# LongmaoTeamTf/deep_recommenders

Measured on AMD Instinct MI355X. Metric: examples/sec/node DeepFM (26 sparse feats, 10M vocab, dim 64), higher is better.
Workload: dtype f32; 1 GPU; DeepFM Criteo-shape synthetic training step (BASELINE.json configs[2]): 26 sparse + 13 dense, 10000000 vocab/field hashed on device, dim 64, DNN [256, 32]+[1] relu, sigmoid-CE, fused SGD; batch 65536 per GPU, ids uniform; tables on one GPU (66.6 GB); gemm_split=f16x2, global_batch=65536, parallelism=single, per_kernel_events=False

## Files before the change

deep_recommenders_amd/csrc/bf3_wgrad.hip:

```cpp
#ifndef DR_NT_WGRAD_GATHER
#define DR_NT_WGRAD_GATHER 0
#endif
#include "bf3_rs_core.h"
#include "tn_rs_reduce.h"

namespace {

using namespace drrs;

struct TnRsArgs {
    const float* X; int64_t ldx;
    const float* Y; int64_t ldy;
    int64_t R; int32_t F; int32_t N;
    int64_t per; int32_t split;
    float* partial; float* colsum;
    const int32_t* ids_t; const int64_t* row_base; const float* table; int32_t nf; const float* dense_pad;
    const uint32_t* x_amax; const uint32_t* x2_amax; const uint32_t* y_amax;
    uint32_t* hdr;
};

template <int GATHER, int H2 = 0>
__global__ __launch_bounds__(512, 2) void bf3_gemm_tn_rs_kernel(TnRsArgs g) {
    constexpr int NW = 8, BMF = 32 * NW, BN = 256, NT = BN / 32;
    constexpr int NPL = RS_NPL<H2>, B_PLANE = RS_B_PLANE, STAGE = RS_STAGE<H2>;
    __shared__ __attribute__((aligned(1024))) unsigned char smem[2 * STAGE];

    const int tid = threadIdx.x, lane = tid & 63;
    const int wave = __builtin_amdgcn_readfirstlane(tid >> 6);
    const int l31 = lane & 31, hi = lane >> 5;
    const int tiles_n = (g.N + BN - 1) / BN, tiles_f = (g.F + BMF - 1) / BMF;
    const int per_slice = tiles_f * tiles_n;
    const int Fp = tiles_f * BMF, Np = tiles_n * BN;
    const int lid = xcd_remap(blockIdx.x, per_slice * g.split);
    const int slice = lid / per_slice, t = lid % per_slice;
    const int f0 = (t / tiles_n) * BMF, n0 = (t % tiles_n) * BN;
    const int64_t r_begin = (int64_t)slice * g.per;
    int64_t r_end = r_begin + g.per;
    if (r_end > g.R) r_end = g.R;
    const int nk = (int)((r_end - r_begin + BK - 1) / BK);
    const bool want_cs = g.colsum != nullptr && f0 == 0;
    float h2_sx = 1.f, h2_sy = 1.f;
    if constexpr (H2) {
        float inv;
        h2_prologue(g.x_amax, g.x2_amax, g.y_amax, h2_sx, h2_sy, inv);
        if (lid == 0 && tid == 0) {
            g.hdr[0] = max(g.x_amax[0], g.x2_amax != nullptr ? g.x2_amax[0] : 0u);
            g.hdr[1] = g.y_amax[0];
        }
    }

    const int fcol = min(f0 + wave * 32 + l31, g.F - 1);
    const int ncol = min(n0 + wave * 32 + l31, g.N - 1);
    const unsigned lds0 = (unsigned)(uintptr_t)(lds_ptr_t)smem;
    const int sw = tn_img_swizzle(l31);
    unsigned b_addr[2];
#pragma unroll
    for (int s = 0; s < 2; ++s) b_addr[s] = rs_frag_addr(lds0, l31, hi, sw, s);
    unsigned char* const wrow = smem + (wave * 32 + l31) * 64;

    float xa[16], yb[16];
    const unsigned xoff = (unsigned)((16 * hi * g.ldx + fcol) * 4), yoff = (unsigned)((16 * hi * g.ldy + ncol) * 4);
    auto load_raw = [&](float (&dst)[16], const float* base, int64_t ld, unsigned voff, int64_t r0) {
        if (r0 + BK <= r_end) {
            const char* rowp = reinterpret_cast<const char*>(base + r0 * ld);
#pragma unroll
            for (int e = 0; e < 16; ++e) dst[e] = *reinterpret_cast<const float*>(rowp + (int64_t)e * ld * 4 + voff);
        } else {
#pragma unroll
            for (int e = 0; e < 16; ++e) {
                const int64_t r = r0 + 16 * hi + e;
                const bool ok = r < r_end;
                const float v = *reinterpret_cast<const float*>(reinterpret_cast<const char*>(base + (ok ? r : r_end - 1) * ld) +
                                                                (voff - (unsigned)(16 * hi * ld * 4)));
                dst[e] = ok ? v : 0.f;
            }
        }
    };
    const int c0w = f0 + wave * 32;
    const bool w_field = GATHER && c0w < 64 * g.nf;
    const bool w_dense = GATHER && !w_field && g.dense_pad != nullptr && c0w < 64 * g.nf + 32;
    const float* gptr = g.table;
    unsigned gpitch = 0;
    const int32_t* idrow = nullptr;
    if (GATHER) {
        if (w_field) {
            const int fld = c0w >> 6;
            const int64_t rbv = g.row_base[fld];
            const int64_t rb = (int64_t)(((uint64_t)(uint32_t)__builtin_amdgcn_readfirstlane((int)(rbv >> 32)) << 32) |
                                         (uint32_t)__builtin_amdgcn_readfirstlane((int)rbv));
            gptr = g.table + rb * 64 + (c0w & 32);
            gpitch = 256;
            idrow = g.ids_t + (int64_t)fld * g.R;
        } else if (w_dense) {
            gptr = g.dense_pad;
            gpitch = 128;
        }
    }
    const __amdgpu_buffer_rsrc_t grsrc =
        __builtin_amdgcn_make_buffer_rsrc(const_cast<float*>(gptr), 0, (w_field || w_dense) ? (int)0xFFFFFF00u : 0, 0x00020000);
    const unsigned gcol = (unsigned)l31 * 4u;
    const int id_lane = (lane & 15) + 16 * hi;
    int idv = 0;
    auto gather_id = [&](int ids_of_tile, int e) -> int {
        switch (e) {
#define GATHER_ID(E) case E: return __builtin_amdgcn_update_dpp(0, ids_of_tile, 0x150 + E, 0xf, 0xf, false);
            GATHER_ID(0) GATHER_ID(1) GATHER_ID(2) GATHER_ID(3) GATHER_ID(4) GATHER_ID(5) GATHER_ID(6) GATHER_ID(7)
            GATHER_ID(8) GATHER_ID(9) GATHER_ID(10) GATHER_ID(11) GATHER_ID(12) GATHER_ID(13) GATHER_ID(14)
#undef GATHER_ID
            default: return __builtin_amdgcn_update_dpp(0, ids_of_tile, 0x15f, 0xf, 0xf, false);
        }
    };
    auto load_ids = [&](int64_t r0) -> int {
        if (!w_field) return 0;
        const int64_t r = r0 + id_lane < g.R ? r0 + id_lane : g.R - 1;
        return idrow[r];
    };
    auto load_gather = [&](float (&dst)[16], int ids_of_tile, int64_t r0) {
        const bool full = r0 + BK <= r_end;
        unsigned off[16];
        if (w_field) {
#pragma unroll
            for (int e = 0; e < 16; ++e) off[e] = (unsigned)gather_id(ids_of_tile, e) * gpitch;
        } else {
            const unsigned o0 = (unsigned)(r0 + 16 * hi) * gpitch;
#pragma unroll
            for (int e = 0; e < 16; ++e) off[e] = o0 + (unsigned)e * gpitch;
        }
        if (!full) {
            const int nv = (int)(r_end - r0 < BK ? r_end - r0 : BK) - 16 * hi;
#pragma unroll
            for (int e = 0; e < 16; ++e) off[e] = e < nv ? off[e] : 0xFFFFFF00u;
        }
#pragma unroll
        for (int e = 0; e < 16; ++e)
            dst[e] = __builtin_bit_cast(float, __builtin_amdgcn_raw_buffer_load_b32(grsrc, (int)(off[e] + gcol), 0, DR_NT_WGRAD_GATHER ? 2 : 0));
    };
    bf16x8 fa[2][3];
    bf16x8 fb[4][3];
    float cs = 0.f;
    auto stage_b = [&](int stage) {
        if (want_cs) {
#pragma unroll
            for (int e = 0; e < 16; ++e) cs += yb[e];
        }
#pragma unroll
        for (int s = 0; s < 2; ++s) {
            bf16x8 p0, p1, p2;
            float v[8];
#pragma unroll
            for (int j = 0; j < 8; ++j) v[j] = yb[8 * s + j];
            if constexpr (H2) h2_split8v(v, h2_sy, p0, p1);
            else rs_split8v(v, p0, p1, p2);
            unsigned char* w = wrow + stage * STAGE + rs_chunk_off(hi, sw, s);
            *reinterpret_cast<bf16x8*>(w) = p0;
            *reinterpret_cast<bf16x8*>(w + B_PLANE) = p1;
            if constexpr (!H2) *reinterpret_cast<bf16x8*>(w + 2 * B_PLANE) = p2;
        }
    };
    auto read_b = [&](int buf, int stage, int q) {
        const unsigned bb = b_addr[q >> 3] + stage * STAGE;
        rs_read_frag<NPL>(fb[buf], bb, q & 7);
    };
    f32x16 acc[NT];
#pragma unroll
    for (int tt = 0; tt < NT; ++tt)
#pragma unroll
        for (int k = 0; k < 16; ++k) acc[tt][k] = 0.f;

    load_raw(yb, g.Y, g.ldy, yoff, r_begin);
    stage_b(0);
    if (GATHER) {
        idv = load_ids(r_begin);
        load_gather(xa, idv, r_begin);
        idv = load_ids(r_begin + BK);
    } else {
        load_raw(xa, g.X, g.ldx, xoff, r_begin);
    }
    load_raw(yb, g.Y, g.ldy, yoff, r_begin + BK);
    asm volatile("s_waitcnt lgkmcnt(0)\n\ts_barrier" ::: "memory");
    read_b(0, 0, 0);
    read_b(1, 0, 1);

    for (int kt = 0; kt < nk; ++kt) {
        const int stage = kt & 1;
        {
            float v[8];
#pragma unroll
            for (int s = 0; s < 2; ++s) {
#pragma unroll
                for (int j = 0; j < 8; ++j) v[j] = xa[8 * s + j];
                if constexpr (H2) h2_split8v(v, h2_sx, fa[s][0], fa[s][1]);
                else rs_split8v(v, fa[s][0], fa[s][1], fa[s][2]);
            }
        }
        if (kt + 1 < nk) stage_b(stage ^ 1);
        __builtin_amdgcn_sched_barrier(0);
        if (GATHER) {
            load_gather(xa, idv, r_begin + (int64_t)(kt + 1) * BK);
            idv = load_ids(r_begin + (int64_t)(kt + 2) * BK);
        } else {
            load_raw(xa, g.X, g.ldx, xoff, r_begin + (int64_t)(kt + 1) * BK);
        }
        load_raw(yb, g.Y, g.ldy, yoff, r_begin + (int64_t)(kt + 2) * BK);
        __builtin_amdgcn_sched_barrier(0);
#pragma unroll
        for (int q = 0; q < 16; ++q) {
            if (q < 14) {
                rs_wait_frag<NPL, NPL>(fb[q & 3]);
                read_b((q + 2) & 3, stage, q + 2);
            } else if (q == 14) {
                rs_wait_frag<NPL, 0>(fb[2]);
                asm volatile("s_barrier" ::: "memory");
                if (kt + 1 < nk) read_b(0, stage ^ 1, 0);
            } else {
                if (kt + 1 < nk) read_b(1, stage ^ 1, 1);
            }
            __builtin_amdgcn_sched_barrier(0);
#pragma unroll
            for (int term = 0; term < RS_TERMS<H2>; ++term) acc[q & 7] = rs_mma_term<H2>(term, fa[q >> 3], fb[q & 3], acc[q & 7]);
            __builtin_amdgcn_sched_barrier(0);
        }
    }
    float* out = g.partial + ((int64_t)slice * Fp + f0 + wave * 32 + 4 * hi) * Np + n0 + l31;
#pragma unroll
    for (int nt = 0; nt < NT; ++nt)
#pragma unroll
        for (int reg = 0; reg < 16; ++reg) out[(int64_t)((reg & 3) + 8 * (reg >> 2)) * Np + nt * 32] = acc[nt][reg];
    if (want_cs) {
        cs += __shfl_xor(cs, 32, 64);
        if (hi == 0) g.colsum[(int64_t)slice * Np + n0 + wave * 32 + l31] = cs;
    }
}

template <int V>
__global__ __launch_bounds__(TN_RS_RED_THREADS) void bf3_tn_rs_reduce_kernel(TnRsApply a) {
    tn_rs_reduce_block<V>(a, blockIdx.x, threadIdx.x);
}

void launch_tn_rs_reduce(const TnRsApply& a, dr_stream_t stream) {
    const int nlb = tn_rs_reduce_blocks(a.F, a.N, a.vec);
    if (a.vec) hipLaunchKernelGGL(bf3_tn_rs_reduce_kernel<4>, dim3(nlb), dim3(TN_RS_RED_THREADS), 0, dr_s(stream), a);
    else hipLaunchKernelGGL(bf3_tn_rs_reduce_kernel<1>, dim3(nlb), dim3(TN_RS_RED_THREADS), 0, dr_s(stream), a);
}
}

void drrs::tn_rs_plan(int64_t R, int32_t F, int32_t N, int& split, int64_t& per, int& Fp, int& Np) {
    const int tf = (F + 255) / 256, tn = (N + 255) / 256;
    Fp = tf * 256;
    Np = tn * 256;
    int64_t sp = 256 / ((int64_t)tf * tn);
    const int64_t max_split = (R + 16 * BK - 1) / (16 * BK);
    if (sp > max_split) sp = max_split;
    if (sp < 1) sp = 1;
    per = ((R + sp - 1) / sp + BK - 1) / BK * BK;
    split = (int)((R + per - 1) / per);
}

extern "C" int64_t dr_bf3_wgrad_workspace_bytes(int64_t R, int32_t F, int32_t N) {
    if (R <= 0 || F <= 0 || N <= 0) return 0;
    int split, Fp, Np;
    int64_t per;
    tn_rs_plan(R, F, N, split, per, Fp, Np);
    return ((int64_t)split * Fp * Np + (int64_t)split * Np + TN_RS_HDR_WORDS) * (int64_t)sizeof(float);
}

static int wgrad_impl(const float* x, int64_t ld_x, const float* dy, int64_t ld_dy, int64_t R, int32_t F, int32_t N,
                      float scale, float* dstW, int64_t ld_w, float* dstb, void* workspace, int64_t workspace_bytes,
                      dr_stream_t stream, const uint32_t* x_amax = nullptr, const uint32_t* dy_amax = nullptr) {
    if (R <= 0 || F <= 0 || N <= 0) return DR_EINVAL;
    if (!x || !dy || !dstW || !workspace || ld_x < F || ld_dy < N || ld_w < N) return DR_EINVAL;
    if (workspace_bytes < dr_bf3_wgrad_workspace_bytes(R, F, N)) return DR_EINVAL;
    int split, Fp, Np;
    int64_t per;
    tn_rs_plan(R, F, N, split, per, Fp, Np);
    const bool h2 = x_amax != nullptr;
    const TnRsApply ap = tn_rs_apply_of(workspace, split, F, N, Fp, Np, h2, scale, dstW, ld_w, dstb);
    TnRsArgs g{x, ld_x, dy, ld_dy, R, F, N, per, split, const_cast<float*>(ap.partial), const_cast<float*>(ap.colsum), nullptr, nullptr, nullptr, 0,
               nullptr, x_amax, nullptr, dy_amax, const_cast<uint32_t*>(ap.hdr)};
    const int grid = (Fp / 256) * (Np / 256) * split;
    if (h2) hipLaunchKernelGGL((bf3_gemm_tn_rs_kernel<0, 1>), dim3(grid), dim3(512), 0, dr_s(stream), g);
    else hipLaunchKernelGGL((bf3_gemm_tn_rs_kernel<0, 0>), dim3(grid), dim3(512), 0, dr_s(stream), g);
    launch_tn_rs_reduce(ap, stream);
    DR_CHECK_LAUNCH();
    return DR_OK;
}

extern "C" int dr_bf3_wgrad(const float* x, int64_t ld_x, const float* dy, int64_t ld_dy, int64_t R, int32_t F, int32_t N,
                            float scale, float* dstW, int64_t ld_w, float* dstb, void* workspace, int64_t workspace_bytes,
                            dr_stream_t stream) {
    return wgrad_impl(x, ld_x, dy, ld_dy, R, F, N, scale, dstW, ld_w, dstb, workspace, workspace_bytes, stream);
}

extern "C" int dr_h2_wgrad(const float* x, int64_t ld_x, const uint32_t* x_amax, const float* dy, int64_t ld_dy, const uint32_t* dy_amax,
                           int64_t R, int32_t F, int32_t N, float scale, float* dstW, int64_t ld_w, float* dstb, void* workspace,
                           int64_t workspace_bytes, dr_stream_t stream) {
    if (!x_amax || !dy_amax) return DR_EINVAL;
    return wgrad_impl(x, ld_x, dy, ld_dy, R, F, N, scale, dstW, ld_w, dstb, workspace, workspace_bytes, stream, x_amax, dy_amax);
}

static int wgrad_emb_impl(const int32_t* ids_t, int64_t R, int32_t nf, const int64_t* row_base, const float* table, int32_t D,
                          const float* dense_pad, const float* dy, int64_t ld_dy, int32_t F, int32_t N, float scale, float* dstW,
                          int64_t ld_w, float* dstb, void* workspace, int64_t workspace_bytes, int32_t parts, dr_stream_t stream,
                          const uint32_t* table_amax = nullptr, const uint32_t* dense_amax = nullptr, const uint32_t* dy_amax = nullptr) {
    if (R <= 0 || F <= 0 || N <= 0 || nf <= 0) return DR_EINVAL;
    if (table_amax != nullptr && (!dy_amax || (F > 64 * nf && !dense_amax))) return DR_EINVAL;
    if (D != 64 || F < 64 * nf || F > 64 * nf + 32) return DR_ESHAPE;
    if (!ids_t || !row_base || !table || !dy || !dstW || !workspace || ld_dy < N || ld_w < N) return DR_EINVAL;
    if (F > 64 * nf && !dense_pad) return DR_EINVAL;
    if (workspace_bytes < dr_bf3_wgrad_workspace_bytes(R, F, N)) return DR_EINVAL;
    int split, Fp, Np;
    int64_t per;
    tn_rs_plan(R, F, N, split, per, Fp, Np);
    const bool h2 = table_amax != nullptr;
    const TnRsApply ap = tn_rs_apply_of(workspace, split, F, N, Fp, Np, h2, scale, dstW, ld_w, dstb);
    TnRsArgs g{nullptr, 0, dy, ld_dy, R, F, N, per, split, const_cast<float*>(ap.partial), const_cast<float*>(ap.colsum), ids_t, row_base, table,
               nf, F > 64 * nf ? dense_pad : nullptr, table_amax, F > 64 * nf ? dense_amax : nullptr, dy_amax, const_cast<uint32_t*>(ap.hdr)};
    const int grid = (Fp / 256) * (Np / 256) * split;
    if (parts & 1) {
        if (h2) hipLaunchKernelGGL((bf3_gemm_tn_rs_kernel<1, 1>), dim3(grid), dim3(512), 0, dr_s(stream), g);
        else hipLaunchKernelGGL((bf3_gemm_tn_rs_kernel<1, 0>), dim3(grid), dim3(512), 0, dr_s(stream), g);
    }
    if (parts & 2) launch_tn_rs_reduce(ap, stream);
    DR_CHECK_LAUNCH();
    return DR_OK;
}

extern "C" int dr_bf3_wgrad_emb(const int32_t* ids_t, int64_t R, int32_t nf, const int64_t* row_base, const float* table, int32_t D,
                                const float* dense_pad, const float* dy, int64_t ld_dy, int32_t F, int32_t N, float scale, float* dstW,
                                int64_t ld_w, float* dstb, void* workspace, int64_t workspace_bytes, int32_t parts, dr_stream_t stream) {
    if (parts < 1 || parts > 3) return DR_EINVAL;
    return wgrad_emb_impl(ids_t, R, nf, row_base, table, D, dense_pad, dy, ld_dy, F, N, scale, dstW, ld_w, dstb, workspace, workspace_bytes,
                          parts, stream);
}

extern "C" int dr_h2_wgrad_emb(const int32_t* ids_t, int64_t R, int32_t nf, const int64_t* row_base, const float* table, int32_t D,
                               const uint32_t* table_amax, const float* dense_pad, const uint32_t* dense_amax, const float* dy, int64_t ld_dy,
                               const uint32_t* dy_amax, int32_t F, int32_t N, float scale, float* dstW, int64_t ld_w, float* dstb,
                               void* workspace, int64_t workspace_bytes, int32_t parts, dr_stream_t stream) {
    if (parts < 1 || parts > 3 || !table_amax || !dy_amax) return DR_EINVAL;
    return wgrad_emb_impl(ids_t, R, nf, row_base, table, D, dense_pad, dy, ld_dy, F, N, scale, dstW, ld_w, dstb, workspace, workspace_bytes,
                          parts, stream, table_amax, dense_amax, dy_amax);
}
```

Baseline: 75.08 million examples/sec.

## Interleave A/B global loads and splits into MFMA groups for f16x2 wgrad path

For the H2 (f16x2) variant of the TN reduce-scatter wgrad GEMM, the main loop runs over full K tiles with unguarded loads, and the single partial tail tile moves into a separate epilogue. The A-tile gather and split are cut into two halves, and the B staging plus next-tile loads are issued from inside the MFMA group loop at fixed q positions. This spreads memory latency and VALU split work across the matrix ops instead of bunching them before the MFMA block. It adds code complexity and register pressure, and it changes load order relative to the LDS barrier.

```diff
diff --git a/deep_recommenders_amd/csrc/bf3_wgrad.hip b/deep_recommenders_amd/csrc/bf3_wgrad.hip
--- a/deep_recommenders_amd/csrc/bf3_wgrad.hip
+++ b/deep_recommenders_amd/csrc/bf3_wgrad.hip
@@ -60,14 +60,14 @@
 
     float xa[16], yb[16];
     const unsigned xoff = (unsigned)((16 * hi * g.ldx + fcol) * 4), yoff = (unsigned)((16 * hi * g.ldy + ncol) * 4);
-    auto load_raw = [&](float (&dst)[16], const float* base, int64_t ld, unsigned voff, int64_t r0) {
-        if (r0 + BK <= r_end) {
+    auto load_raw = [&](float (&dst)[16], const float* base, int64_t ld, unsigned voff, int64_t r0, int e0 = 0, int e1 = 16, bool known_full = false) {
+        if (known_full || r0 + BK <= r_end) {
             const char* rowp = reinterpret_cast<const char*>(base + r0 * ld);
 #pragma unroll
-            for (int e = 0; e < 16; ++e) dst[e] = *reinterpret_cast<const float*>(rowp + (int64_t)e * ld * 4 + voff);
+            for (int e = e0; e < e1; ++e) dst[e] = *reinterpret_cast<const float*>(rowp + (int64_t)e * ld * 4 + voff);
         } else {
 #pragma unroll
-            for (int e = 0; e < 16; ++e) {
+            for (int e = e0; e < e1; ++e) {
                 const int64_t r = r0 + 16 * hi + e;
                 const bool ok = r < r_end;
                 const float v = *reinterpret_cast<const float*>(reinterpret_cast<const char*>(base + (ok ? r : r_end - 1) * ld) +
@@ -115,25 +115,31 @@
         const int64_t r = r0 + id_lane < g.R ? r0 + id_lane : g.R - 1;
         return idrow[r];
     };
-    auto load_gather = [&](float (&dst)[16], int ids_of_tile, int64_t r0) {
-        const bool full = r0 + BK <= r_end;
-        unsigned off[16];
+    auto gather_offsets = [&](unsigned (&off)[16], int ids_of_tile, int64_t r0, int e0, int e1, bool known_full = false) {
+        const bool full = known_full || r0 + BK <= r_end;
         if (w_field) {
 #pragma unroll
-            for (int e = 0; e < 16; ++e) off[e] = (unsigned)gather_id(ids_of_tile, e) * gpitch;
+            for (int e = e0; e < e1; ++e) off[e] = (unsigned)gather_id(ids_of_tile, e) * gpitch;
         } else {
             const unsigned o0 = (unsigned)(r0 + 16 * hi) * gpitch;
 #pragma unroll
-            for (int e = 0; e < 16; ++e) off[e] = o0 + (unsigned)e * gpitch;
+            for (int e = e0; e < e1; ++e) off[e] = o0 + (unsigned)e * gpitch;
         }
         if (!full) {
             const int nv = (int)(r_end - r0 < BK ? r_end - r0 : BK) - 16 * hi;
 #pragma unroll
-            for (int e = 0; e < 16; ++e) off[e] = e < nv ? off[e] : 0xFFFFFF00u;
-        }
-#pragma unroll
-        for (int e = 0; e < 16; ++e)
+            for (int e = e0; e < e1; ++e) off[e] = e < nv ? off[e] : 0xFFFFFF00u;
+        }
+    };
+    auto gather_issue = [&](float (&dst)[16], const unsigned (&off)[16], int e0, int e1) {
+#pragma unroll
+        for (int e = e0; e < e1; ++e)
             dst[e] = __builtin_bit_cast(float, __builtin_amdgcn_raw_buffer_load_b32(grsrc, (int)(off[e] + gcol), 0, DR_NT_WGRAD_GATHER ? 2 : 0));
+    };
+    auto load_gather = [&](float (&dst)[16], int ids_of_tile, int64_t r0) {
+        unsigned off[16];
+        gather_offsets(off, ids_of_tile, r0, 0, 16);
+        gather_issue(dst, off, 0, 16);
     };
     bf16x8 fa[2][3];
     bf16x8 fb[4][3];
@@ -167,58 +173,145 @@
 #pragma unroll
         for (int k = 0; k < 16; ++k) acc[tt][k] = 0.f;
 
-    load_raw(yb, g.Y, g.ldy, yoff, r_begin);
-    stage_b(0);
-    if (GATHER) {
-        idv = load_ids(r_begin);
-        load_gather(xa, idv, r_begin);
-        idv = load_ids(r_begin + BK);
-    } else {
-        load_raw(xa, g.X, g.ldx, xoff, r_begin);
-    }
-    load_raw(yb, g.Y, g.ldy, yoff, r_begin + BK);
-    asm volatile("s_waitcnt lgkmcnt(0)\n\ts_barrier" ::: "memory");
-    read_b(0, 0, 0);
-    read_b(1, 0, 1);
-
-    for (int kt = 0; kt < nk; ++kt) {
-        const int stage = kt & 1;
-        {
-            float v[8];
-#pragma unroll
-            for (int s = 0; s < 2; ++s) {
-#pragma unroll
-                for (int j = 0; j < 8; ++j) v[j] = xa[8 * s + j];
-                if constexpr (H2) h2_split8v(v, h2_sx, fa[s][0], fa[s][1]);
-                else rs_split8v(v, fa[s][0], fa[s][1], fa[s][2]);
-            }
-        }
-        if (kt + 1 < nk) stage_b(stage ^ 1);
-        __builtin_amdgcn_sched_barrier(0);
-        if (GATHER) {
-            load_gather(xa, idv, r_begin + (int64_t)(kt + 1) * BK);
-            idv = load_ids(r_begin + (int64_t)(kt + 2) * BK);
-        } else {
-            load_raw(xa, g.X, g.ldx, xoff, r_begin + (int64_t)(kt + 1) * BK);
-        }
-        load_raw(yb, g.Y, g.ldy, yoff, r_begin + (int64_t)(kt + 2) * BK);
-        __builtin_amdgcn_sched_barrier(0);
+    auto split_a = [&](int s) {
+        float v[8];
+#pragma unroll
+        for (int j = 0; j < 8; ++j) v[j] = xa[8 * s + j];
+        if constexpr (H2) h2_split8v(v, h2_sx, fa[s][0], fa[s][1]);
+        else rs_split8v(v, fa[s][0], fa[s][1], fa[s][2]);
+    };
+    auto mma_groups = [&](int stage, bool more, auto&& before_group) {
 #pragma unroll
         for (int q = 0; q < 16; ++q) {
+            before_group(q);
             if (q < 14) {
                 rs_wait_frag<NPL, NPL>(fb[q & 3]);
                 read_b((q + 2) & 3, stage, q + 2);
             } else if (q == 14) {
                 rs_wait_frag<NPL, 0>(fb[2]);
                 asm volatile("s_barrier" ::: "memory");
-                if (kt + 1 < nk) read_b(0, stage ^ 1, 0);
+                if (more) read_b(0, stage ^ 1, 0);
             } else {
-                if (kt + 1 < nk) read_b(1, stage ^ 1, 1);
+                if (more) read_b(1, stage ^ 1, 1);
             }
             __builtin_amdgcn_sched_barrier(0);
 #pragma unroll
             for (int term = 0; term < RS_TERMS<H2>; ++term) acc[q & 7] = rs_mma_term<H2>(term, fa[q >> 3], fb[q & 3], acc[q & 7]);
             __builtin_amdgcn_sched_barrier(0);
+        }
+    };
+    if constexpr (!H2) {
+        load_raw(yb, g.Y, g.ldy, yoff, r_begin);
+        stage_b(0);
+        if (GATHER) {
+            idv = load_ids(r_begin);
+            load_gather(xa, idv, r_begin);
+            idv = load_ids(r_begin + BK);
+        } else {
+            load_raw(xa, g.X, g.ldx, xoff, r_begin);
+        }
+        load_raw(yb, g.Y, g.ldy, yoff, r_begin + BK);
+        asm volatile("s_waitcnt lgkmcnt(0)\n\ts_barrier" ::: "memory");
+        read_b(0, 0, 0);
+        read_b(1, 0, 1);
+        for (int kt = 0; kt < nk; ++kt) {
+            const int stage = kt & 1;
+            split_a(0);
+            split_a(1);
+            if (kt + 1 < nk) stage_b(stage ^ 1);
+            __builtin_amdgcn_sched_barrier(0);
+            if (GATHER) {
+                load_gather(xa, idv, r_begin + (int64_t)(kt + 1) * BK);
+                idv = load_ids(r_begin + (int64_t)(kt + 2) * BK);
+            } else {
+                load_raw(xa, g.X, g.ldx, xoff, r_begin + (int64_t)(kt + 1) * BK);
+            }
+            load_raw(yb, g.Y, g.ldy, yoff, r_begin + (int64_t)(kt + 2) * BK);
+            __builtin_amdgcn_sched_barrier(0);
+            mma_groups(stage, kt + 1 < nk, [](int) {});
+        }
+    } else {
+        constexpr int Q_A1 = 5, Q_B = 10;
+        const int nfull = (int)((r_end - r_begin) / BK);
+        if (nfull > 0) {
+            const int64_t r_last = r_begin + (int64_t)(nfull - 1) * BK;
+            int64_t r1 = nfull > 1 ? r_begin + BK : r_last;
+            int64_t r2 = nfull > 2 ? r_begin + 2 * BK : r_last;
+            load_raw(yb, g.Y, g.ldy, yoff, r_begin, 0, 16, true);
+            stage_b(0);
+            if (GATHER) {
+                idv = load_ids(r_begin);
+                unsigned off[16];
+                gather_offsets(off, idv, r_begin, 0, 16, true);
+                gather_issue(xa, off, 0, 8);
+                __builtin_amdgcn_sched_barrier(0);
+                idv = load_ids(r1);
+                __builtin_amdgcn_sched_barrier(0);
+                gather_issue(xa, off, 8, 16);
+            } else {
+                load_raw(xa, g.X, g.ldx, xoff, r_begin, 0, 16, true);
+            }
+            __builtin_amdgcn_sched_barrier(0);
+            load_raw(yb, g.Y, g.ldy, yoff, r1, 0, 16, true);
+            __builtin_amdgcn_sched_barrier(0);
+            asm volatile("s_waitcnt lgkmcnt(0)\n\ts_barrier" ::: "memory");
+            read_b(0, 0, 0);
+            read_b(1, 0, 1);
+            for (int kt = 0; kt < nfull; ++kt) {
+                const int stage = kt & 1;
+                const bool more = kt + 1 < nfull;
+                split_a(0);
+                __builtin_amdgcn_sched_barrier(0);
+                if (GATHER) {
+                    unsigned off[16];
+                    gather_offsets(off, idv, r1, 0, 8, true);
+                    gather_issue(xa, off, 0, 8);
+                } else {
+                    load_raw(xa, g.X, g.ldx, xoff, r1, 0, 8, true);
+                }
+                __builtin_amdgcn_sched_barrier(0);
+                mma_groups(stage, more, [&](int q) {
+                    if (q == Q_A1) {
+                        split_a(1);
+                        __builtin_amdgcn_sched_barrier(0);
+                        if (GATHER) {
+                            unsigned off[16];
+                            gather_offsets(off, idv, r1, 8, 16, true);
+                            idv = load_ids(r2);
+                            gather_issue(xa, off, 8, 16);
+                        } else {
+                            load_raw(xa, g.X, g.ldx, xoff, r1, 8, 16, true);
+                        }
+                        __builtin_amdgcn_sched_barrier(0);
+                    }
+                    if (q == Q_B) {
+                        if (more) stage_b(stage ^ 1);
+                        __builtin_amdgcn_sched_barrier(0);
+                        load_raw(yb, g.Y, g.ldy, yoff, r2, 0, 16, true);
+                        __builtin_amdgcn_sched_barrier(0);
+                    }
+                });
+                r1 = r2;
+                r2 = r2 < r_last ? r2 + BK : r_last;
+            }
+        }
+        if (nk > nfull) {
+            const int stage = nfull & 1;
+            const int64_t r0 = r_begin + (int64_t)nfull * BK;
+            load_raw(yb, g.Y, g.ldy, yoff, r0);
+            if (GATHER) {
+                idv = load_ids(r0);
+                load_gather(xa, idv, r0);
+            } else {
+                load_raw(xa, g.X, g.ldx, xoff, r0);
+            }
+            stage_b(stage);
+            split_a(0);
+            split_a(1);
+            asm volatile("s_waitcnt lgkmcnt(0)\n\ts_barrier" ::: "memory");
+            read_b(0, stage, 0);
+            read_b(1, stage, 1);
+            mma_groups(stage, false, [](int) {});
         }
     }
     float* out = g.partial + ((int64_t)slice * Fp + f0 + wave * 32 + 4 * hi) * Np + n0 + l31;
```

After: 76.82 million examples/sec (median of 6 runs). 1.02x the previous value.
